# hwang595/ps_pytorch

Measured on AMD Instinct MI355X. Metric: images/sec (whole node), ResNet-18/CIFAR-10 synchronous PS training, higher is better.
Workload: dtype bf16; 1 GPU; model=ResNet18, global_batch=1024, input=3x32x32, per_worker_batch=1024, parallelism=single-gpu, engine=single-machine trainer (hipGraph-captured step), compress_grad=n/a (no comm at N=1), overlap=n/a (no comm at N=1)

## Files before the change

ps_pytorch_amd/ops/__init__.py:

```python
from __future__ import annotations

import ctypes
import os
from pathlib import Path
from typing import Optional

import torch

_LIB: Optional[ctypes.CDLL] = None
_LIB_ERR: Optional[str] = None

PS_F32 = 0
PS_BF16 = 1

_DTYPE_TAG = {torch.float32: PS_F32, torch.bfloat16: PS_BF16}

F32_SYMBOLS = (
    'ps_conv_fwd_f32', 'ps_conv_dgrad_f32', 'ps_conv_wgrad_f32',
    'ps_conv_bias_grad_f32',
    'ps_maxpool_fwd_f32', 'ps_maxpool_bwd_f32',
    'ps_gavgpool_fwd_f32', 'ps_gavgpool_bwd_f32',
    'ps_softmax_ce_fwd_f32', 'ps_softmax_ce_bwd_f32',
    'ps_ce_metrics_f32', 'ps_softmax_ce_fwd_metrics_f32',
)


def _so_path() -> Path:
    return Path(__file__).resolve().parent / "libps_hip.so"


def _try_load() -> None:
    global _LIB, _LIB_ERR
    if _LIB is not None or _LIB_ERR is not None:
        return
    p = _so_path()
    if not p.exists():
        _LIB_ERR = f"{p} not built (run ps_pytorch_amd.ops.build or __graft_entry__.build())"
        return
    try:
        lib = ctypes.CDLL(str(p))
        lib.ps_fused_sgd.argtypes = [
            ctypes.c_void_p, ctypes.c_void_p, ctypes.c_void_p, ctypes.c_void_p,
            ctypes.c_long, ctypes.c_float, ctypes.c_float, ctypes.c_float,
            ctypes.c_float, ctypes.c_int, ctypes.c_int, ctypes.c_int, ctypes.c_void_p]
        lib.ps_pack_bf16.argtypes = [ctypes.c_void_p, ctypes.c_void_p,
                                     ctypes.c_long, ctypes.c_void_p]
        lib.ps_unpack_bf16.argtypes = [ctypes.c_void_p, ctypes.c_void_p,
                                       ctypes.c_long, ctypes.c_void_p]
        lib.ps_pack_q8.argtypes = [ctypes.c_void_p, ctypes.c_void_p,
                                   ctypes.c_long, ctypes.c_int, ctypes.c_void_p]
        lib.ps_pack_q8_ef.argtypes = [ctypes.c_void_p, ctypes.c_void_p,
                                      ctypes.c_void_p, ctypes.c_long,
                                      ctypes.c_int, ctypes.c_void_p]
        lib.ps_pack_bf16_ef.argtypes = [ctypes.c_void_p, ctypes.c_void_p,
                                        ctypes.c_void_p, ctypes.c_long,
                                        ctypes.c_void_p]
        lib.ps_unpack_q8.argtypes = [ctypes.c_void_p, ctypes.c_void_p,
                                     ctypes.c_long, ctypes.c_int, ctypes.c_void_p]
        lib.ps_acc.argtypes = [ctypes.c_void_p, ctypes.c_void_p,
                               ctypes.c_long, ctypes.c_int, ctypes.c_void_p]
        lib.ps_pack_topk_ef.argtypes = [ctypes.c_void_p] * 3 + [
            ctypes.c_long, ctypes.c_int, ctypes.c_int, ctypes.c_void_p]
        lib.ps_pack_topk_ef.restype = ctypes.c_int
        lib.ps_unpack_topk.argtypes = [ctypes.c_void_p, ctypes.c_void_p,
                                       ctypes.c_long, ctypes.c_int,
                                       ctypes.c_int, ctypes.c_void_p]
        lib.ps_unpack_topk.restype = ctypes.c_int
        lib.ps_fanin_reduce.argtypes = [
            ctypes.c_void_p, ctypes.POINTER(ctypes.c_void_p), ctypes.c_int,
            ctypes.c_int, ctypes.c_int, ctypes.c_long, ctypes.c_void_p]
        lib.ps_fanin_reduce.restype = ctypes.c_int
        lib.ps_fanin_sgd.argtypes = [ctypes.c_void_p] * 3 + [
            ctypes.c_int, ctypes.POINTER(ctypes.c_void_p), ctypes.c_int,
            ctypes.c_int, ctypes.c_int, ctypes.c_long] + [
            ctypes.c_float] * 4 + [ctypes.c_int, ctypes.c_void_p]
        lib.ps_fanin_sgd.restype = ctypes.c_int
        lib.ps_conv_fwd.argtypes = [ctypes.c_void_p] * 5 + [ctypes.c_int] * 11 + [ctypes.c_void_p]
        lib.ps_conv_dgrad.argtypes = [ctypes.c_void_p] * 4 + [ctypes.c_int] * 11 + [ctypes.c_void_p]
        lib.ps_conv_wgrad.argtypes = [ctypes.c_void_p] * 4 + [ctypes.c_int] * 12 + [ctypes.c_void_p]
        lib.ps_conv_wgrad_row_variant.argtypes = [ctypes.c_void_p] * 3 + [
            ctypes.c_int] * 9 + [ctypes.c_void_p]
        lib.ps_conv_wgrad_row_variant.restype = ctypes.c_int
        lib.ps_conv_bias_grad.argtypes = [ctypes.c_void_p] * 3 + [
            ctypes.c_long, ctypes.c_int, ctypes.c_void_p]
        lib.ps_wt_transpose.argtypes = [ctypes.c_void_p, ctypes.c_void_p,
                                        ctypes.c_int, ctypes.c_int, ctypes.c_void_p]
        lib.ps_fused_adam.argtypes = [ctypes.c_void_p] * 6 + [
            ctypes.c_long] + [ctypes.c_float] * 7 + [
            ctypes.c_int, ctypes.c_int, ctypes.c_void_p]
        lib.ps_bn_fwd.argtypes = [ctypes.c_void_p] * 13 + [
            ctypes.c_int,
            ctypes.c_long, ctypes.c_long, ctypes.c_float, ctypes.c_float,
            ctypes.c_int, ctypes.c_int, ctypes.c_int, ctypes.c_void_p]
        lib.ps_bn_bwd.argtypes = [ctypes.c_void_p] * 12 + [
            ctypes.c_long, ctypes.c_long, ctypes.c_int, ctypes.c_int,
            ctypes.c_void_p]
        lib.ps_softmax_ce_fwd.argtypes = [ctypes.c_void_p] * 5 + [
            ctypes.c_long, ctypes.c_int, ctypes.c_void_p]
        lib.ps_softmax_ce_bwd.argtypes = [ctypes.c_void_p] * 5 + [
            ctypes.c_long, ctypes.c_int, ctypes.c_void_p]
        lib.ps_ce_metrics.argtypes = [ctypes.c_void_p] * 5 + [
            ctypes.c_long] + [ctypes.c_int] * 6 + [ctypes.c_void_p]
        lib.ps_softmax_ce_fwd_metrics.argtypes = [ctypes.c_void_p] * 7 + [
            ctypes.c_long] + [ctypes.c_int] * 6 + [ctypes.c_void_p]
        lib.ps_maxpool_fwd.argtypes = [ctypes.c_void_p] * 3 + [
            ctypes.c_int] * 10 + [ctypes.c_void_p]
        lib.ps_maxpool_bwd.argtypes = [ctypes.c_void_p] * 3 + [
            ctypes.c_int] * 10 + [ctypes.c_void_p]
        lib.ps_gavgpool_fwd.argtypes = [ctypes.c_void_p] * 2 + [
            ctypes.c_int] * 3 + [ctypes.c_void_p]
        lib.ps_gavgpool_bwd.argtypes = [ctypes.c_void_p] * 2 + [
            ctypes.c_int] * 3 + [ctypes.c_void_p]
        lib.ps_pad4.argtypes = [ctypes.c_void_p, ctypes.c_void_p,
                                ctypes.c_long, ctypes.c_int, ctypes.c_void_p]
        lib.ps_padc.argtypes = [ctypes.c_void_p, ctypes.c_void_p,
                                ctypes.c_long, ctypes.c_int, ctypes.c_int,
                                ctypes.c_void_p]
        lib.ps_act_drop_fwd.argtypes = [ctypes.c_void_p] * 3 + [
            ctypes.c_long, ctypes.c_int, ctypes.c_int, ctypes.c_uint32,
            ctypes.c_float, ctypes.c_uint64, ctypes.c_uint32,
            ctypes.c_void_p, ctypes.c_void_p]
        lib.ps_act_drop_bwd.argtypes = [ctypes.c_void_p] * 3 + [
            ctypes.c_long, ctypes.c_int, ctypes.c_float, ctypes.c_void_p]
        lib.ps_rng_advance.argtypes = [ctypes.c_void_p, ctypes.c_void_p]
        lib.ps_augment_batch.argtypes = [ctypes.c_void_p] * 5 + [
            ctypes.c_long] + [ctypes.c_int] * 7 + [
            ctypes.POINTER(ctypes.c_float), ctypes.POINTER(ctypes.c_float),
            ctypes.c_uint64, ctypes.c_uint32, ctypes.c_void_p,
            ctypes.c_void_p]
        lib.ps_conv_fwd_f32.argtypes = [ctypes.c_void_p] * 4 + [ctypes.c_int] * 11 + [ctypes.c_void_p]
        lib.ps_conv_dgrad_f32.argtypes = [ctypes.c_void_p] * 4 + [ctypes.c_int] * 11 + [ctypes.c_void_p]
        lib.ps_conv_wgrad_f32.argtypes = [ctypes.c_void_p] * 4 + [ctypes.c_int] * 12 + [ctypes.c_void_p]
        lib.ps_conv_bias_grad_f32.argtypes = [ctypes.c_void_p] * 3 + [
            ctypes.c_long, ctypes.c_int, ctypes.c_void_p]
        lib.ps_softmax_ce_fwd_f32.argtypes = lib.ps_softmax_ce_fwd.argtypes
        lib.ps_softmax_ce_bwd_f32.argtypes = lib.ps_softmax_ce_bwd.argtypes
        lib.ps_ce_metrics_f32.argtypes = lib.ps_ce_metrics.argtypes
        lib.ps_softmax_ce_fwd_metrics_f32.argtypes = \
            lib.ps_softmax_ce_fwd_metrics.argtypes
        lib.ps_maxpool_fwd_f32.argtypes = lib.ps_maxpool_fwd.argtypes
        lib.ps_maxpool_bwd_f32.argtypes = lib.ps_maxpool_bwd.argtypes
        lib.ps_gavgpool_fwd_f32.argtypes = lib.ps_gavgpool_fwd.argtypes
        lib.ps_gavgpool_bwd_f32.argtypes = lib.ps_gavgpool_bwd.argtypes
        _LIB = lib
    except OSError as e:
        _LIB_ERR = str(e)


def lib_or_none() -> Optional[ctypes.CDLL]:
    _try_load()
    return _LIB


def require_lib() -> ctypes.CDLL:
    _try_load()
    if _LIB is None:
        raise RuntimeError(
            f"ps_pytorch_amd HIP extension unavailable on a GPU host: {_LIB_ERR}")
    return _LIB


def dtype_tag(dt: torch.dtype) -> int:
    try:
        return _DTYPE_TAG[dt]
    except KeyError:
# ... 9 lines not shown
```

ps_pytorch_amd/ops/kernels/conv.hip:

```cpp
#include "common.h"
#include <stdlib.h>

typedef __bf16 bf16x8_t __attribute__((ext_vector_type(8)));
typedef unsigned short ushort8_t __attribute__((ext_vector_type(8)));
typedef float f32x4_t __attribute__((ext_vector_type(4)));

#define MFMA_BF16(a, b, c) __builtin_amdgcn_mfma_f32_16x16x32_bf16(a, b, c, 0, 0, 0)

union V16 {
    uint4 u4;
    unsigned short us[8];
    bf16x8_t bv;
};

__device__ __forceinline__ V16 zero16() {
    V16 v; v.u4 = make_uint4(0, 0, 0, 0); return v;
}

template <bool AL>
__device__ __forceinline__ V16 load16(const unsigned short* src, int cc, int Cn) {
    V16 v;
    if constexpr (AL) {
        v.u4 = *(const uint4*)src;
    } else if (cc + 8 <= Cn) {
// ... 408 lines not shown
            int col = n0 + segc;
            f32x4_t a0 = *(const f32x4_t*)&sf[rl * TN + segc];
            f32x4_t a1 = *(const f32x4_t*)&sf[rl * TN + segc + 4];
            float v[8];
#pragma unroll
            for (int k2 = 0; k2 < 4; ++k2) { v[k2] = a0[k2]; v[4 + k2] = a1[k2]; }
            if (vec_ok && col + 8 <= Nout) {
                V16 o;
                if constexpr (ACCF) {
                    V16 cv = *(const V16*)&carry[om * Nout + col];
#pragma unroll
                    for (int k2 = 0; k2 < 8; ++k2)
                        v[k2] += bf16_to_f32(cv.us[k2]);
                }
#pragma unroll
                for (int k2 = 0; k2 < 8; ++k2) o.us[k2] = f32_to_bf16(v[k2]);
                if constexpr (STATS)
#pragma unroll
                    for (int k2 = 0; k2 < 8; ++k2) {
                        float rv = bf16_to_f32(o.us[k2]);
                        ssum[k2] += rv;
                        ssq[k2] += rv * rv;
                    }
                *(uint4*)&dst[om * Nout + col] = o.u4;
            } else {
                for (int k2 = 0; k2 < 8 && col + k2 < Nout; ++k2) {
                    float vv = v[k2];
                    if constexpr (ACCF)
                        vv += bf16_to_f32(carry[om * Nout + col + k2]);
                    unsigned short ov = f32_to_bf16(vv);
                    if constexpr (STATS) {
                        float rv = bf16_to_f32(ov);
                        ssum[k2] += rv;
                        ssq[k2] += rv * rv;
                    }
                    dst[om * Nout + col + k2] = ov;
                }
            }
        }
        if constexpr (STATS) {
            __syncthreads();
            float* sp = sf;
#pragma unroll
            for (int k2 = 0; k2 < 8; ++k2) {
                sp[(rl0 * SEG + t % SEG) * 8 + k2] = ssum[k2];
                sp[(RPP * SEG + rl0 * SEG + t % SEG) * 8 + k2] = ssq[k2];
            }
            __syncthreads();
            if (rl0 == 0) {
                for (int rr2 = 1; rr2 < RPP; ++rr2)
#pragma unroll
                    for (int k2 = 0; k2 < 8; ++k2) {
                        ssum[k2] += sp[(rr2 * SEG + t % SEG) * 8 + k2];
                        ssq[k2] += sp[(RPP * SEG + rr2 * SEG + t % SEG) * 8 + k2];
                    }
                float* dst2 = stats + tile_m * 2 * (long)Nout + n0 + segc;
                for (int k2 = 0; k2 < 8 && n0 + segc + k2 < Nout; ++k2) {
                    dst2[k2] = ssum[k2];
                    dst2[Nout + k2] = ssq[k2];
                }
            }
        }
    } else {
#pragma unroll
    for (int nj = 0; nj < NJ; ++nj) {
        int col = n0 + wn * (NJ * 16) + nj * 16 + fr;
        float bv = (!DGRAD && bias && col < Nout) ? bf16_to_f32(bias[col]) : 0.f;
#pragma unroll
        for (int mi = 0; mi < 4; ++mi)
#pragma unroll
        for (int e = 0; e < 4; ++e) {
            long om = m0 + wm * 64 + mi * 16 + fq * 4 + e;
            if (om < M && col < Nout) {
                float v = acc[mi][nj][e] + bv;
                if constexpr (ACCF)
                    v += bf16_to_f32(carry[om * Nout + col]);
                dst[om * Nout + col] = f32_to_bf16(v);
            }
        }
    }
    }
}

template <int TM, int TN, bool AL = true, int SWZM = 2, bool ACCF = false>
__global__ __launch_bounds__(256) void conv_dgrad2_kernel(
    const unsigned short* __restrict__ dout,
    const unsigned short* __restrict__ wgt,
    unsigned short* __restrict__ dx,
    const unsigned short* __restrict__ carry,
    int Nb, int H, int W, int C, int K, int P, int Q,
    int R, int S, int pad, int4 ends, int4 codes)
{
    int bx = blockIdx.x;
    int cls;
    if      (bx < ends.x) cls = 0;
    else if (bx < ends.y) { cls = 1; bx -= ends.x; }
    else if (bx < ends.z) { cls = 2; bx -= ends.y; }
    else                  { cls = 3; bx -= ends.z; }
    const int code = (cls == 0) ? codes.x : (cls == 1) ? codes.y
                     : (cls == 2) ? codes.z : codes.w;
    const int hp = code >> 1, wp = code & 1;
    const int Hc = (H - hp + 1) >> 1, Wc = (W - wp + 1) >> 1;
    __shared__ __attribute__((aligned(16))) FwdLds<TM, TN> lds;
    constexpr int SWZ = SWZM;
    constexpr int AR = TM / 32;
    constexpr int BR = TN / 32;
    const long M = (long)Nb * Hc * Wc;
    const int tiles_n = (C + TN - 1) / TN;
    const long m0 = (bx / tiles_n) * (long)TM;
    const int n0 = (bx % tiles_n) * TN;
    const int t = threadIdx.x;
    const int trow = t >> 3;
    const int cc8 = (t & 7) * 8;

    const int r0 = (hp + pad) & 1, s0 = (wp + pad) & 1;
    const int nr = (R > r0) ? ((R - r0 + 1) >> 1) : 0;
    const int ns = (S > s0) ? ((S - s0 + 1) >> 1) : 0;

    const unsigned short* pA[AR];
    unsigned int vm[AR];
#pragma unroll
    for (int rr = 0; rr < AR; ++rr) {
        long m = m0 + trow + 32 * rr;
        pA[rr] = dout; vm[rr] = 0;
        if (m < M) {
            int n = (int)(m / ((long)Hc * Wc)); int rem = (int)(m % ((long)Hc * Wc));
            int h = hp + 2 * (rem / Wc), w = wp + 2 * (rem % Wc);
            int p1 = (h + pad - r0) >> 1, q1 = (w + pad - s0) >> 1;
            pA[rr] = dout + (long)n * P * Q * K + ((long)p1 * Q + q1) * K + cc8;
            unsigned int msk = 0;
            for (int ri = 0; ri < nr; ++ri)
                for (int si = 0; si < ns; ++si)
                    if (p1 - ri >= 0 && p1 - ri < P
                        && q1 - si >= 0 && q1 - si < Q)
                        msk |= 1u << (ri * ns + si);
            vm[rr] = msk;
        }
    }

    constexpr int WGM = TM / 64;
    constexpr int WGN = 4 / WGM;
    constexpr int NJ = TN / WGN / 16;
    const int lane = t & 63, wid = t >> 6;
    const int wm = (WGN == 1) ? wid : (wid >> 1);
    const int wn = (WGN == 1) ? 0 : (wid & 1);
    const int fr = lane & 15, fq = lane >> 4;
    f32x4_t acc[4][NJ];
#pragma unroll
    for (int i = 0; i < 4; ++i)
#pragma unroll
        for (int j = 0; j < NJ; ++j) acc[i][j] = {0.f, 0.f, 0.f, 0.f};

    const int KC = (K + 63) >> 6;
    const int KCm1 = (KC - 1) * 64;
    const int nsteps = nr * ns * KC;
    int lsi = 0, lkc = 0;
    V16 areg[AR], breg[BR];

    const unsigned short* pB[BR];
    bool colv[BR];
#pragma unroll
    for (int rr = 0; rr < BR; ++rr) {
        int col = n0 + trow + 32 * rr;
        colv[rr] = col < C;
        pB[rr] = wgt + (((long)(r0 * S + s0) * C) + (colv[rr] ? col : 0))
                 * (long)K + cc8;
// ... 498 lines not shown
#pragma unroll
            for (int mi = 0; mi < MI; ++mi)
#pragma unroll
                for (int nj = 0; nj < 2; ++nj)
                    acc[s][mi][nj] = MFMA_BF16(a[mi].v, bf[nj].v,
                                               acc[s][mi][nj]);
        }
    };

    load_step();
    write_lds(0);
    if (nsteps > 1) load_step();
    __syncthreads();
    int it = 0;
    for (; it + 3 < nsteps; it += 2) {
        write_lds(1);
        load_step();
        mfma_step(0);
        __syncthreads();
        write_lds(0);
        load_step();
        mfma_step(1);
        __syncthreads();
    }
    const int rem = nsteps - it;
    if (rem >= 2) {
        write_lds(1);
        if (rem >= 3) load_step();
    }
    if (rem >= 1) mfma_step(0);
    if (rem >= 2) {
        __syncthreads();
        if (rem >= 3) write_lds(0);
        mfma_step(1);
    }
    if (rem >= 3) {
        __syncthreads();
        mfma_step(0);
    }

    const int RSC = 9 * C;
    float* dstp = partial + (long)sid * K * RSC;
#pragma unroll
    for (int s = 0; s < 3; ++s)
#pragma unroll
    for (int mi = 0; mi < MI; ++mi)
#pragma unroll
    for (int nj = 0; nj < 2; ++nj)
#pragma unroll
    for (int e = 0; e < 4; ++e) {
        int k = k0 + wm * (MI * 16) + mi * 16 + fq * 4 + e;
        int c = c0 + wn * 32 + nj * 16 + fr;
        if (k < K && c < C)
            dstp[(long)k * RSC + (r * 3 + s) * C + c] = acc[s][mi][nj][e];
    }
}


__device__ __forceinline__ int wrho(int e) {
    return (((e >> 1) & 1) + ((e >> 3) & 1) * 2) << 1;
}

#define WG_RING_NST 4

struct WgRingStage {
    unsigned short A[32][64];
    unsigned short B[64][64];
};

__device__ __forceinline__ void wg_ring_dma3(
    const void* g0, const void* g1, const void* g2,
    unsigned l0, unsigned l1, unsigned l2)
{
    unsigned keep;
    asm volatile(
        "s_mov_b32 %0, m0\n\t"
        "s_mov_b32 m0, %4\n\ts_nop 0\n\tglobal_load_lds_dwordx4 %1, off\n\t"
        "s_mov_b32 m0, %5\n\ts_nop 0\n\tglobal_load_lds_dwordx4 %2, off\n\t"
        "s_mov_b32 m0, %6\n\ts_nop 0\n\tglobal_load_lds_dwordx4 %3, off\n\t"
        "s_mov_b32 m0, %0"
        : "=&s"(keep)
        : "v"(g0), "v"(g1), "v"(g2), "s"(l0), "s"(l1), "s"(l2)
        : "memory");
}

template <int N>
__device__ __forceinline__ void wg_ring_sync() {
    asm volatile("s_waitcnt vmcnt(%0)\n\ts_waitcnt lgkmcnt(0)\n\ts_barrier"
                 :: "i"(N) : "memory");
}

template <int NST>
__global__ __launch_bounds__(256) void conv_wgrad_row_ring_kernel(
    const unsigned short* __restrict__ dout,
    const unsigned short* __restrict__ in,
    float* __restrict__ partial,
    const unsigned short* __restrict__ zpage,
    int Nb, int H, int W, int C, int K, int P, int Q,
    int split, int ipr, int l2q, int l2p, int per_xcd)
{
    static_assert(NST == 3 || NST == 4, "ring depth");
    constexpr int TK = 64;
    constexpr int PAD = 1;
    constexpr int DPS = 3;
    const int ROWS = 32 >> l2q;
    const int HW2 = W + 2;
    __shared__ __attribute__((aligned(16))) WgRingStage sg0, sg1, sg2, sg3;
    auto stg = [&](int st) -> WgRingStage* {
        return st == 0 ? &sg0 : st == 1 ? &sg1 : st == 2 ? &sg2 : &sg3;
    };
    constexpr int MI = TK / 32;
    const int tiles_k = (K + TK - 1) / TK;
    const int tiles_c = (C + 63) >> 6;
    long l = (long)(blockIdx.x & 7) * per_xcd + (blockIdx.x >> 3);
    const long nlog = (long)tiles_k * tiles_c * 3 * split;
    if (l >= nlog) return;
    int b = (int)l;
    const int k0 = (b % tiles_k) * TK; b /= tiles_k;
    const int c0 = (b % tiles_c) * 64; b /= tiles_c;
    const int r = b % 3; b /= 3;
    const int sid = b;
    const long rows_total = (long)Nb * P;
    const long row0 = (long)sid * ipr;
    const long row1 = (row0 + ipr < rows_total) ? row0 + ipr : rows_total;

    const int t = threadIdx.x;
    const int lane = t & 63, wid = t >> 6;
    const int wm = wid >> 1, wn = wid & 1;
    const int fr = lane & 15, fq = lane >> 4;
    f32x4_t acc[3][MI][2];
#pragma unroll
    for (int si = 0; si < 3; ++si)
#pragma unroll
        for (int i = 0; i < MI; ++i)
#pragma unroll
            for (int j = 0; j < 2; ++j) acc[si][i][j] = {0.f, 0.f, 0.f, 0.f};

    const int nsteps = (int)((row1 - row0 + (1 << (5 - l2q)) - 1)
                             >> (5 - l2q));

    const int apix = wid * 8 + (lane >> 3);
    const int aoct = ((lane & 7) ^ wrho(apix));
    const unsigned short* pdout = dout + (row0 << l2q) * K + k0;
    const int a_off = apix * K + aoct * 8;
    const int a_row = apix >> l2q;
    const long inrow0 = row0 + r - PAD;
    const unsigned short* pin0 = in + inrow0 * W * C + c0;
    int b_rib[2], b_off[2];
    bool b_wok[2];
#pragma unroll
    for (int j = 0; j < 2; ++j) {
        int hp = wid * 16 + j * 8 + (lane >> 3);
        int oct = ((lane & 7) ^ wrho(hp));
        b_rib[j] = hp / HW2;
        int wpx = hp - b_rib[j] * HW2 - 1;
        b_wok[j] = wpx >= 0 && wpx < W && hp < ROWS * HW2;
        b_off[j] = (b_rib[j] * W + (wpx < 0 ? 0 : wpx)) * C + oct * 8;
    }
    long prow = row0;

    const unsigned wu = (unsigned)__builtin_amdgcn_readfirstlane(wid);
    const unsigned ldA = wu * (8 * 128);
    const unsigned ldB = (unsigned)sizeof(sg0.A) + wu * (16 * 128);

    auto dma_stage = [&](int st) {
        const unsigned sb = (unsigned)(unsigned long)
            (__attribute__((address_space(3))) void*)stg(st);
        const unsigned short* gs[DPS];
        const long rl = rows_total - prow;
        const int rleft = rl < 64 ? (int)rl : 64;
        const int pl = (int)prow;
        gs[0] = a_row < rleft ? pdout + a_off : zpage;
#pragma unroll
        for (int j = 0; j < 2; ++j) {
            int h = ((pl + b_rib[j]) & (P - 1)) + r - PAD;
            bool ok = b_wok[j] & ((unsigned)h < (unsigned)H)
                      & (b_rib[j] < rleft);
            gs[1 + j] = ok ? pin0 + b_off[j] : zpage;
        }
        wg_ring_dma3(gs[0], gs[1], gs[2],
                     sb + ldA, sb + ldB, sb + ldB + 8 * 128);
        pdout += (long)32 * K;
        pin0 += (long)ROWS * W * C;
        prow += ROWS;
    };

    const char* lb0 = (const char*)&sg0;
    unsigned roA[MI][2];
    unsigned roB[3][2][2];
#pragma unroll
    for (int i = 0; i < 2; ++i) {
        int e = fq * 8 + i * 4 + (fr >> 2);
        int qd = fr & 3;
#pragma unroll
        for (int mi = 0; mi < MI; ++mi) {
            int o = (wm * MI + mi) * 2 + (qd >> 1);
            roA[mi][i] = (unsigned)((char*)&sg0.A[e]
                             [(o ^ wrho(e)) * 8 + (qd & 1) * 4] - lb0);
        }
        int rib = e >> l2q, q = e & (Q - 1);
#pragma unroll
        for (int si = 0; si < 3; ++si) {
            int hp = rib * HW2 + q + si;
#pragma unroll
            for (int nj = 0; nj < 2; ++nj) {
                int o = (wn * 2 + nj) * 2 + (qd >> 1);
                roB[si][nj][i] = (unsigned)((char*)&sg0.B[hp]
                                 [(o ^ wrho(hp)) * 8 + (qd & 1) * 4] - lb0);
            }
        }
    }

    union U64x8 { bf16x4_t h[2]; bf16x8_t v; };
    auto mfma_step = [&](int st) {
        const char* sbp = (const char*)stg(st);
        U64x8 a[MI];
#pragma unroll
        for (int mi = 0; mi < MI; ++mi) {
            a[mi].h[0] = ds_tr16p((const unsigned short*)
                (sbp + roA[mi][0]));
            a[mi].h[1] = ds_tr16p((const unsigned short*)
                (sbp + roA[mi][1]));
        }
#pragma unroll
        for (int si = 0; si < 3; ++si) {
            U64x8 bf[2];
#pragma unroll
            for (int nj = 0; nj < 2; ++nj) {
                bf[nj].h[0] = ds_tr16p((const unsigned short*)
                    (sbp + roB[si][nj][0]));
                bf[nj].h[1] = ds_tr16p((const unsigned short*)
                    (sbp + roB[si][nj][1]));
            }
#pragma unroll
            for (int mi = 0; mi < MI; ++mi)
#pragma unroll
                for (int nj = 0; nj < 2; ++nj)
                    acc[si][mi][nj] = MFMA_BF16(a[mi].v, bf[nj].v,
                                                acc[si][mi][nj]);
        }
    };

    auto ring_sync = [&](int ahead) {
        if (NST > 3 && ahead >= 2) wg_ring_sync<2 * DPS>();
        else if (ahead >= 1)       wg_ring_sync<DPS>();
        else                       wg_ring_sync<0>();
    };

#pragma unroll
    for (int j = 0; j < NST - 1; ++j)
        if (j < nsteps) dma_stage(j);
    int it = 0;
    for (; it + 2 * NST - 2 < nsteps; it += NST) {
#pragma unroll
        for (int j = 0; j < NST; ++j) {
            ring_sync(NST - 2);
            dma_stage((j + NST - 1) % NST);
            mfma_step(j);
        }
    }
    const int rem = nsteps - it;
#pragma unroll
    for (int j = 0; j < 2 * NST - 2; ++j) {
        if (j < rem) {
            const int left = rem - 1 - j;
            ring_sync(left < NST - 2 ? left : NST - 2);
            if (j + NST - 1 < rem) dma_stage((j + NST - 1) % NST);
            mfma_step(j % NST);
        }
    }

    const int RSC = 9 * C;
    float* dstp = partial + (long)sid * K * RSC;
#pragma unroll
    for (int si = 0; si < 3; ++si)
#pragma unroll
    for (int mi = 0; mi < MI; ++mi)
#pragma unroll
    for (int nj = 0; nj < 2; ++nj)
#pragma unroll
    for (int e = 0; e < 4; ++e) {
        int k = k0 + wm * (MI * 16) + mi * 16 + fq * 4 + e;
        int c = c0 + wn * 32 + nj * 16 + fr;
        if (k < K && c < C)
            dstp[(long)k * RSC + (r * 3 + si) * C + c] = acc[si][mi][nj][e];
    }
}

template <int STRIDE, bool POW2, bool AL = true, int CPM = 0>
__global__ __launch_bounds__(256) void conv_wgrad_small_kernel(
    const unsigned short* __restrict__ dout,
    const unsigned short* __restrict__ in,
    float* __restrict__ partial,
    int Nb, int H, int W, int C, int K, int P, int Q,
    int R, int S, int pad, int split, int chunk,
    int l2pq, int l2q,
    unsigned long long mpq, unsigned long long mq)
{
    __shared__ __attribute__((aligned(16))) WgradLds<64> lds;
    const long M = (long)Nb * P * Q;
    const int RSC = R * S * C;
    const int tiles_k = (K + 63) >> 6;
    const int nc = (RSC + 63) >> 6;
    int b = blockIdx.x;
    const int k0 = (b % tiles_k) * 64; b /= tiles_k;
    const int e0 = (b % nc) * 64; b /= nc;
    const int sid = b;
    const long mbeg = (long)sid * chunk;
    const long mend = (mbeg + chunk < M) ? mbeg + chunk : M;

    const int t = threadIdx.x;
    const int trow = t >> 3;
    const int cc8 = (t & 7) * 8;
    const int lane = t & 63, wid = t >> 6;
    const int wm = wid >> 1, wn = wid & 1;
    const int fr = lane & 15, fq = lane >> 4;
    f32x4_t acc[2][2];
#pragma unroll
    for (int i = 0; i < 2; ++i)
#pragma unroll
        for (int j = 0; j < 2; ++j) acc[i][j] = {0.f, 0.f, 0.f, 0.f};

    int tre[8], tse[8], toff[8];
#pragma unroll
    for (int u = 0; u < 8; ++u) {
        int e = e0 + cc8 + u;
        if constexpr (CPM == 8) {
            int tp = e / C;
            tre[u] = tp / S;
// ... 351 lines not shown
    int vec_ok = (((uintptr_t)dst | (uintptr_t)src) & 15) == 0;
    int blocks;
    ew_grid(vec_ok ? ((n + 7) >> 3) / PS_SEED_U + 1 : n, 256, &blocks);
    hipLaunchKernelGGL(seed_dx_kernel<PS_SEED_U>, dim3(blocks), dim3(256), 0,
                       (hipStream_t)strm, (unsigned short*)dst,
                       (const unsigned short*)src, n, vec_ok);
}


static inline int swz_mode() {
    static int m = -1;
    if (m < 0) { const char* e = getenv("PS_SWZ"); m = e ? atoi(e) : 2; }
    return m;
}

static inline int glds_mode() {
    static int m = -1;
    if (m < 0) { const char* e = getenv("PS_GLDS"); m = e ? atoi(e) : 1; }
    return m;
}

static const unsigned short* zpage_ptr() {
    static const unsigned short* z = [] {
        void* p = nullptr;
        (void)hipMalloc(&p, 128);
        (void)hipMemset(p, 0, 128);
        return (const unsigned short*)p;
    }();
    return z;
}

#define LAUNCH_GEMM(TM, TN, ST, DG, SM) LAUNCH_GEMM_NB(TM, TN, ST, DG, SM, 2)
#define LAUNCH_GEMM_NB(TM, TN, ST, DG, SM, NBV)                               \
    do {                                                                      \
        if (swz_mode() == 1) LAUNCH_GEMM_SW(TM, TN, ST, DG, SM, NBV, 1, false); \
        else                 LAUNCH_GEMM_SW(TM, TN, ST, DG, SM, NBV, 2, false); \
    } while (0)
#define LAUNCH_GEMM_ACC(TM, TN, ST, DG, SM, ACV)                              \
    do {                                                                      \
        if (swz_mode() == 1) LAUNCH_GEMM_SW(TM, TN, ST, DG, SM, 2, 1, ACV);   \
        else                 LAUNCH_GEMM_SW(TM, TN, ST, DG, SM, 2, 2, ACV);   \
    } while (0)
#define LAUNCH_GEMM_CV(TM, TN, ST, SM, NBV) LAUNCH_GEMM_CP(TM, TN, ST, SM, NBV, 4)
#define LAUNCH_GEMM_CP(TM, TN, ST, SM, NBV, CPV)                              \
    do {                                                                      \
        long M_ = (long)Nb * P * Q;                                           \
        long grid = ((M_ + TM - 1) / TM) * ((K + TN - 1) / TN);               \
        hipLaunchKernelGGL((conv_gemm_kernel<TM, TN, ST, false, SM, ALV, NBV, \
                                             2, false, CPV>),               \
            dim3((unsigned)grid), dim3(256), 0, (hipStream_t)strm,            \
            (const unsigned short*)src, (const unsigned short*)wgt,           \
            (const unsigned short*)bias, (unsigned short*)dst,                \
            (const unsigned short*)carry, nullptr, nullptr,                   \
            Nb, H, W, C, K, P, Q, R, S, pad);                                 \
    } while (0)
#define LAUNCH_GEMM_GLS(TM, TN, ST, DG, SM, NBV, SWV, ACV, GLV, STV)          \
    do {                                                                      \
        long M_ = DG ? (long)Nb * H * W : (long)Nb * P * Q;                   \
        int Nout_ = DG ? C : K;                                               \
        long grid = ((M_ + TM - 1) / TM) * ((Nout_ + TN - 1) / TN);           \
        hipLaunchKernelGGL((conv_gemm_kernel<TM, TN, ST, DG, SM, ALV, NBV,    \
                                             SWV, ACV, 0, GLV, STV>),         \
            dim3((unsigned)grid), dim3(256), 0, (hipStream_t)strm,            \
            (const unsigned short*)src, (const unsigned short*)wgt,           \
            (const unsigned short*)bias, (unsigned short*)dst,                \
            (const unsigned short*)carry, zpage_ptr(), (float*)stats,         \
            Nb, H, W, C, K, P, Q, R, S, pad);                                 \
    } while (0)
#define LAUNCH_GEMM_GL(TM, TN, ST, DG, SM, NBV, SWV, ACV, GLV)                \
    do {                                                                      \
        if (!(DG) && stats) LAUNCH_GEMM_GLS(TM, TN, ST, DG, SM, NBV, SWV, ACV, GLV, true); \
        else                LAUNCH_GEMM_GLS(TM, TN, ST, DG, SM, NBV, SWV, ACV, GLV, false); \
    } while (0)
#define LAUNCH_GEMM_SW(TM, TN, ST, DG, SM, NBV, SWV, ACV)                     \
    do {                                                                      \
        if constexpr (ALV && !(SM)) {                                         \
            if (glds_mode()) LAUNCH_GEMM_GL(TM, TN, ST, DG, SM, NBV, SWV, ACV, true); \
            else             LAUNCH_GEMM_GL(TM, TN, ST, DG, SM, NBV, SWV, ACV, false); \
        } else {                                                              \
            LAUNCH_GEMM_GL(TM, TN, ST, DG, SM, NBV, SWV, ACV, false);         \
        }                                                                     \
    } while (0)

extern "C" void ps_conv_fwd(
    const void* src, const void* wgt, const void* bias, void* dst,
    void* stats,
    int Nb, int H, int W, int C, int K, int P, int Q,
    int R, int S, int stride, int pad, void* strm)
{
    const void* carry = nullptr;
    bool al = (C & 63) == 0;
#define FWD_BODY()                                                            \
    do {                                                                      \
        if (R * S > 1 && C == 4 && R * S * 4 <= 64) {        \
            if (K <= 32) {            \
                if (stride == 1) LAUNCH_GEMM_CV(128, 32, 1, true, 1);         \
                else             LAUNCH_GEMM_CV(128, 32, 2, true, 1);         \
            } else if (stride == 1) LAUNCH_GEMM_CV(128, 64, 1, true, 1);      \
            else             LAUNCH_GEMM_CV(128, 64, 2, true, 1);             \
        } else if (R * S > 1 && C == 4 && R * S * 4 <= 256) {                 \
            if (K <= 32) {                                                    \
                if (stride == 1) LAUNCH_GEMM_CV(128, 32, 1, true, 2);         \
                else             LAUNCH_GEMM_CV(128, 32, 2, true, 2);         \
            } else if (stride == 1) LAUNCH_GEMM_CV(128, 64, 1, true, 2);      \
            else             LAUNCH_GEMM_CV(128, 64, 2, true, 2);             \
        } else if (R * S > 1 && (C & 7) == 0 && (C & 63)                      \
                   && R * S * C <= 768) {              \
            if (K <= 32) {                                                    \
                if (stride == 1) LAUNCH_GEMM_CP(128, 32, 1, true, 2, 8);      \
                else             LAUNCH_GEMM_CP(128, 32, 2, true, 2, 8);      \
            } else if (stride == 1) LAUNCH_GEMM_CP(128, 64, 1, true, 2, 8);   \
            else             LAUNCH_GEMM_CP(128, 64, 2, true, 2, 8);          \
        } else if (R * S > 1 && R * S * C <= 64) {    \
            if (stride == 1) LAUNCH_GEMM_NB(128, 64, 1, false, true, 1);      \
            else             LAUNCH_GEMM_NB(128, 64, 2, false, true, 1);      \
        } else if (R * S > 1 && R * S * C <= 192) {                           \
            if (stride == 1) LAUNCH_GEMM(128, 64, 1, false, true);            \
            else             LAUNCH_GEMM(128, 64, 2, false, true);            \
        } else if (R * S == 1 && C <= 64) {              \
            if (stride == 1) LAUNCH_GEMM_NB(128, 64, 1, false, false, 1);     \
            else             LAUNCH_GEMM_NB(128, 64, 2, false, false, 1);     \
        } else if (K >= 128) {                                                \
            if (stride == 1) LAUNCH_GEMM(128, 128, 1, false, false);          \
            else             LAUNCH_GEMM(128, 128, 2, false, false);          \
        } else if (K <= 32) {         \
            if (stride == 1) LAUNCH_GEMM(128, 32, 1, false, false);           \
            else             LAUNCH_GEMM(128, 32, 2, false, false);           \
        } else {                                                              \
            if (stride == 1) LAUNCH_GEMM(128, 64, 1, false, false);           \
            else             LAUNCH_GEMM(128, 64, 2, false, false);           \
        }                                                                     \
    } while (0)
    if (al) { constexpr bool ALV = true; FWD_BODY(); }
    else    { constexpr bool ALV = false; FWD_BODY(); }
#undef FWD_BODY
}

extern "C" void ps_conv_dgrad(
    const void* src, const void* wgt, void* dst, const void* carry,
    int Nb, int H, int W, int C, int K, int P, int Q,
    int R, int S, int stride, int pad, void* strm)
{
    const void* bias = nullptr;
    const void* stats = nullptr;
    bool al = (K & 63) == 0;
    if (stride == 1) {
#define DG_BODY(ACV)                                                          \
        do {                                                                  \
            if (C >= 128)     LAUNCH_GEMM_ACC(128, 128, 1, true, false, ACV); \
            else if (C <= 32) LAUNCH_GEMM_ACC(128, 32, 1, true, false, ACV);  \
            else              LAUNCH_GEMM_ACC(128, 64, 1, true, false, ACV);  \
        } while (0)
        if (al) { constexpr bool ALV = true;
                  if (carry) DG_BODY(true); else DG_BODY(false); }
        else    { constexpr bool ALV = false;
                  if (carry) DG_BODY(true); else DG_BODY(false); }
#undef DG_BODY
    } else {
        const unsigned short* dout = (const unsigned short*)src;
        bool any_empty = false;
        for (int hp = 0; hp < 2 && hp < H; ++hp)
        for (int wp = 0; wp < 2 && wp < W; ++wp) {
            int r0 = (hp + pad) & 1, s0 = (wp + pad) & 1;
            if (R <= r0 || S <= s0) any_empty = true;
        }
        if (any_empty)
            launch_seed_dx(dst, carry, (long)Nb * H * W * C, strm);
        int TM_ = 128, TN_ = (C >= 128) ? 128 : 64;
        int tiles_n_ = (C + TN_ - 1) / TN_;
        int ends_[4] = {0, 0, 0, 0}, codes_[4] = {0, 0, 0, 0};
        int slot = 0, total = 0;
        for (int hp = 0; hp < 2 && hp < H; ++hp)
        for (int wp = 0; wp < 2 && wp < W; ++wp) {
            int r0 = (hp + pad) & 1, s0 = (wp + pad) & 1;
            if (R <= r0 || S <= s0) continue;
            int Hc = (H - hp + 1) >> 1, Wc = (W - wp + 1) >> 1;
            long M_ = (long)Nb * Hc * Wc;
            total += (int)(((M_ + TM_ - 1) / TM_) * tiles_n_);
            ends_[slot] = total;
            codes_[slot] = (hp << 1) | wp;
            ++slot;
        }
        for (int i = slot; i < 4; ++i) { ends_[i] = total; codes_[i] = 0; }
        if (total == 0) return;
        int4 ends = make_int4(ends_[0], ends_[1], ends_[2], ends_[3]);
        int4 codes = make_int4(codes_[0], codes_[1], codes_[2], codes_[3]);
#define DG2_SW(TM, TN, ALV, SWV, ACV)                                         \
        hipLaunchKernelGGL((conv_dgrad2_kernel<TM, TN, ALV, SWV, ACV>),       \
            dim3((unsigned)total), dim3(256), 0, (hipStream_t)strm, dout,     \
            (const unsigned short*)wgt, (unsigned short*)dst,                 \
            (const unsigned short*)carry,                                     \
            Nb, H, W, C, K, P, Q, R, S, pad, ends, codes)
#define DG2_AC(TM, TN, ALV, SWV) do {                                         \
        if (carry) DG2_SW(TM, TN, ALV, SWV, true);                            \
        else       DG2_SW(TM, TN, ALV, SWV, false); } while (0)
#define DG2(TM, TN, ALV) do {                                                 \
        if (swz_mode() == 1) DG2_AC(TM, TN, ALV, 1);                          \
        else                 DG2_AC(TM, TN, ALV, 2); } while (0)
        if (al) { if (C >= 128) DG2(128, 128, true);
                  else          DG2(128, 64, true); }
        else    { if (C >= 128) DG2(128, 128, false);
                  else          DG2(128, 64, false); }
#undef DG2
    }
}

static inline int ilog2_exact(long v) {
    int l = 0; while ((1L << l) < v) ++l;
    return ((1L << l) == v) ? l : -1;
}

static bool wgrad_row_eligible(int H, int W, int C, int K, int P, int Q,
                               int variant)
{
    if (P != H || Q != W || ilog2_exact(Q) < 0 || ilog2_exact(P) < 0
        || Q < 4 || Q > 32)
        return false;
    if (variant == 1) return (C & 63) == 0 && (K & 63) == 0;
    return variant == 0;
}

static void launch_wgrad_row(
    const void* dout, const void* in, void* partial_f32,
    int Nb, int H, int W, int C, int K, int P, int Q, int split,
    int variant, void* strm)
{
    const int TKr = 64;
    int l2q_ = ilog2_exact(Q);
    int tkr = (K + TKr - 1) / TKr, tcr = (C + 63) / 64;
    long rows_total = (long)Nb * P;
    int ROWS = 32 >> l2q_;
    long ipr_l = (rows_total + split - 1) / split;
    ipr_l = ((ipr_l + ROWS - 1) / ROWS) * ROWS;
    long nlog = (long)tkr * tcr * 3 * split;
    int pxc = (int)((nlog + 7) / 8);
    long grid_r = (long)pxc * 8;
    bool alr = ((C & 63) == 0) && (K % TKr == 0);
#define WGR(TKV, ALV)                                                         \
    hipLaunchKernelGGL((conv_wgrad_row_kernel<TKV, ALV>),                     \
        dim3((unsigned)grid_r), dim3(256), 0, (hipStream_t)strm,              \
        (const unsigned short*)dout, (const unsigned short*)in,               \
        (float*)partial_f32, Nb, H, W, C, K, P, Q,                            \
        split, (int)ipr_l, l2q_, 0, pxc)
    if (variant == 1)
        hipLaunchKernelGGL((conv_wgrad_row_ring_kernel<WG_RING_NST>),
            dim3((unsigned)grid_r), dim3(256), 0, (hipStream_t)strm,
            (const unsigned short*)dout, (const unsigned short*)in,
            (float*)partial_f32, zpage_ptr(), Nb, H, W, C, K, P, Q,
            split, (int)ipr_l, l2q_, 0, pxc);
    else if (alr) WGR(64, true);
    else          WGR(64, false);
#undef WGR
}

extern "C" int ps_conv_wgrad_row_variant(
    const void* dout, const void* in, void* partial_f32,
    int Nb, int H, int W, int C, int K, int P, int Q, int split,
    int variant, void* strm)
{
    if (split < 1 || Nb < 1
        || !wgrad_row_eligible(H, W, C, K, P, Q, variant))
        return 1;
    launch_wgrad_row(dout, in, partial_f32, Nb, H, W, C, K, P, Q, split,
                     variant, strm);
    return 0;
}

extern "C" void ps_conv_wgrad(
    const void* dout, const void* in, void* partial_f32, void* dw,
    int Nb, int H, int W, int C, int K, int P, int Q,
    int R, int S, int stride, int pad, int split, void* strm)
{
    long M = (long)Nb * P * Q;
    long chunk64 = (M + (long)split * 64 - 1) / ((long)split * 64);
    int chunk = (int)(chunk64 * 64);
    if (R * S > 1 && ((C == 4 && R * S * 4 <= 256)
                      || ((C & 7) == 0 && (C & 63) && R * S * C <= 768)
                      || R * S * C <= 192)) {
        int tiles_k = (K + 63) / 64;
        int nc_s = (R * S * C + 63) / 64;
        long grid_s = (long)tiles_k * nc_s * split;
        int l2pq_ = ilog2_exact((long)P * Q), l2q_ = ilog2_exact(Q);
        bool pw = l2pq_ >= 0 && l2q_ >= 0;
        unsigned long long mpq_ = fdiv_magic((long)P * Q);
        unsigned long long mq_ = fdiv_magic(Q);
#define WGS(ST, PW, CV)                                                       \
        hipLaunchKernelGGL((conv_wgrad_small_kernel<ST, PW, false, CV>),      \
// ... 115 lines not shown
```

Baseline: 130,300 images/sec.

## Add halo-tiled 3x3 conv kernel for 64-channel fwd and dgrad

Adds a dedicated 3x3 stride-1 conv kernel for C=K=64 layers at 16 or 32 width. It loads each 128-pixel output tile plus its one-pixel halo into LDS once through direct global-to-LDS DMA, then reuses that tile across all nine taps. Weight taps stream through a three-slot ring buffer overlapped with the MFMA work. This replaces the generic implicit-GEMM path, which re-gathers input for every tap. The cost is extra code, LDS pressure that may limit occupancy, and a new path selected by default through an env var.

```diff
diff --git a/ps_pytorch_amd/ops/__init__.py b/ps_pytorch_amd/ops/__init__.py
--- a/ps_pytorch_amd/ops/__init__.py
+++ b/ps_pytorch_amd/ops/__init__.py
@@ -81,6 +81,9 @@
         lib.ps_conv_wgrad_row_variant.argtypes = [ctypes.c_void_p] * 3 + [
             ctypes.c_int] * 9 + [ctypes.c_void_p]
         lib.ps_conv_wgrad_row_variant.restype = ctypes.c_int
+        lib.ps_conv_halo_variant.argtypes = [ctypes.c_int] + [
+            ctypes.c_void_p] * 5 + [ctypes.c_int] * 8 + [ctypes.c_void_p]
+        lib.ps_conv_halo_variant.restype = ctypes.c_int
         lib.ps_conv_bias_grad.argtypes = [ctypes.c_void_p] * 3 + [
             ctypes.c_long, ctypes.c_int, ctypes.c_void_p]
         lib.ps_wt_transpose.argtypes = [ctypes.c_void_p, ctypes.c_void_p,
diff --git a/ps_pytorch_amd/ops/kernels/conv.hip b/ps_pytorch_amd/ops/kernels/conv.hip
--- a/ps_pytorch_amd/ops/kernels/conv.hip
+++ b/ps_pytorch_amd/ops/kernels/conv.hip
@@ -514,6 +514,201 @@
     }
 }
 
+template <int W>
+struct HaloLds {
+    static constexpr int RT = 128 / W;
+    static constexpr int HW2 = W + 2;
+    static constexpr int NPIX = (RT + 2) * HW2;
+    static constexpr int PW = (NPIX + 31) / 32;
+    unsigned short A[PW * 32][64];
+    unsigned short B[3][64][64];
+};
+
+__device__ __forceinline__ void halo_dma1(const void* g0, unsigned l0)
+{
+    unsigned keep;
+    asm volatile(
+        "s_mov_b32 %0, m0\n\t"
+        "s_mov_b32 m0, %2\n\ts_nop 0\n\tglobal_load_lds_dwordx4 %1, off\n\t"
+        "s_mov_b32 m0, %0"
+        : "=&s"(keep) : "v"(g0), "s"(l0) : "memory");
+}
+
+__device__ __forceinline__ void halo_dma2(
+    const void* g0, const void* g1, unsigned l0, unsigned l1)
+{
+    unsigned keep;
+    asm volatile(
+        "s_mov_b32 %0, m0\n\t"
+        "s_mov_b32 m0, %3\n\ts_nop 0\n\tglobal_load_lds_dwordx4 %1, off\n\t"
+        "s_mov_b32 m0, %4\n\ts_nop 0\n\tglobal_load_lds_dwordx4 %2, off\n\t"
+        "s_mov_b32 m0, %0"
+        : "=&s"(keep) : "v"(g0), "v"(g1), "s"(l0), "s"(l1) : "memory");
+}
+
+template <int N>
+__device__ __forceinline__ void lds_ring_sync() {
+    asm volatile("s_waitcnt vmcnt(%0)\n\ts_waitcnt lgkmcnt(0)\n\ts_barrier"
+                 :: "i"(N) : "memory");
+}
+
+template <int W, bool DGRAD, bool ACCF>
+__global__ __launch_bounds__(256) void conv3x3_halo_kernel(
+    const unsigned short* __restrict__ src,
+    const unsigned short* __restrict__ wgt,
+    const unsigned short* __restrict__ bias,
+    unsigned short* __restrict__ dst,
+    const unsigned short* __restrict__ carry,
+    const unsigned short* __restrict__ zpage,
+    int H)
+{
+    using L = HaloLds<W>;
+    constexpr int RT = L::RT, HW2 = L::HW2, NPIX = L::NPIX, PW = L::PW;
+    constexpr int J0 = 5;
+    static_assert(RT * HW2 <= 32 * J0 && 32 * PW - 2 * HW2 <= 32 * J0
+                  && J0 <= PW, "early-start piece count");
+    static_assert(sizeof(L) >= 128 * 64 * 4, "f32 staging fits LDS");
+    __shared__ __attribute__((aligned(128))) L lds;
+
+    const int t = threadIdx.x;
+    const int lane = t & 63, wid = t >> 6;
+    const int wm = wid >> 1, wn = wid & 1;
+    const int fr = lane & 15, fq = lane >> 4;
+    const int tpi = H / RT;
+    const int n = blockIdx.x / tpi;
+    const int h0 = (blockIdx.x - n * tpi) * RT;
+    const long m0 = (long)blockIdx.x * 128;
+    const unsigned short* img = src + (long)n * H * W * 64;
+
+    const int wu = __builtin_amdgcn_readfirstlane(wid);
+    const unsigned ldsA = (unsigned)(unsigned long)
+        (__attribute__((address_space(3))) void*)&lds.A[0][0];
+    const unsigned ldsB = (unsigned)(unsigned long)
+        (__attribute__((address_space(3))) void*)&lds.B[0][0][0];
+
+    const unsigned short* pB[2];
+#pragma unroll
+    for (int rr = 0; rr < 2; ++rr) {
+        int row = wid * 16 + rr * 8 + (lane >> 3);
+        pB[rr] = wgt + row * (DGRAD ? 64 : 9 * 64)
+                 + gswz<2>(row, lane & 7) * 8;
+    }
+    constexpr int BTAP = DGRAD ? 64 * 64 : 64;
+    auto dma_b = [&](int tap) {
+        const unsigned l = ldsB + (tap % 3) * 8192 + wu * 2048;
+        halo_dma2(pB[0] + tap * BTAP, pB[1] + tap * BTAP, l, l + 1024);
+    };
+    auto dma_a = [&](int j) {
+        const int i = j * 4 + wu;
+        const int gi = DGRAD ? 4 * PW - 1 - i : i;
+        const int lp = gi * 8 + (lane >> 3);
+        const int hr = lp / HW2, hc = lp - hr * HW2;
+        const int h = h0 - 1 + hr, wc = hc - 1;
+        const bool ok = (lp < NPIX) & ((unsigned)h < (unsigned)H)
+                        & ((unsigned)wc < (unsigned)W);
+        const int off = (h * W + wc) * 64
+                        + (((lane & 7) ^ (((lp >> 1) & 3) << 1)) * 8);
+        const unsigned short* gs = ok ? img + off : zpage;
+        halo_dma1(gs, ldsA + gi * 1024);
+    };
+
+    f32x4_t acc[4][2];
+#pragma unroll
+    for (int i = 0; i < 4; ++i)
+#pragma unroll
+        for (int j = 0; j < 2; ++j) acc[i][j] = {0.f, 0.f, 0.f, 0.f};
+
+    int lp0[4];
+#pragma unroll
+    for (int mi = 0; mi < 4; ++mi) {
+        int o = wm * 64 + mi * 16 + fr;
+        lp0[mi] = (o / W) * HW2 + (o % W);
+    }
+    int brow[2];
+#pragma unroll
+    for (int nj = 0; nj < 2; ++nj) brow[nj] = wn * 32 + nj * 16 + fr;
+
+    auto mfma_tap = [&](int tap) {
+        const int r = tap / 3, s = tap % 3;
+        const int toff = DGRAD ? (2 - r) * HW2 + (2 - s) : r * HW2 + s;
+#pragma unroll
+        for (int kk = 0; kk < 2; ++kk) {
+            bf16x8_t a[4], b[2];
+#pragma unroll
+            for (int mi = 0; mi < 4; ++mi) {
+                int lp = lp0[mi] + toff;
+                a[mi] = *(const bf16x8_t*)
+                    &lds.A[lp][((kk * 4 + fq) ^ (((lp >> 1) & 3) << 1)) * 8];
+            }
+#pragma unroll
+            for (int nj = 0; nj < 2; ++nj)
+                b[nj] = *(const bf16x8_t*)
+                    &lds.B[tap % 3][brow[nj]]
+                          [gswz<2>(brow[nj], kk * 4 + fq) * 8];
+#pragma unroll
+            for (int mi = 0; mi < 4; ++mi)
+#pragma unroll
+                for (int nj = 0; nj < 2; ++nj)
+                    acc[mi][nj] = MFMA_BF16(a[mi], b[nj], acc[mi][nj]);
+        }
+    };
+
+    dma_b(0);
+#pragma unroll
+    for (int j = 0; j < J0; ++j) dma_a(j);
+    dma_b(1);
+#pragma unroll
+    for (int j = J0; j < PW; ++j) dma_a(j);
+    dma_b(2);
+
+#pragma unroll
+    for (int tap = 0; tap < 9; ++tap) {
+        if (tap == 0)      lds_ring_sync<PW - J0 + 4>();
+        else if (tap == 1) lds_ring_sync<PW - J0 + 2>();
+        else if (tap < 8)  lds_ring_sync<2>();
+        else               lds_ring_sync<0>();
+        if (tap >= 1 && tap + 2 < 9) dma_b(tap + 2);
+        mfma_tap(tap);
+    }
+    lds_ring_sync<0>();
+
+    float* sf = reinterpret_cast<float*>(&lds);
+#pragma unroll
+    for (int nj = 0; nj < 2; ++nj) {
+        int cl = wn * 32 + nj * 16 + fr;
+        float bv = (!DGRAD && bias) ? bf16_to_f32(bias[cl]) : 0.f;
+#pragma unroll
+        for (int mi = 0; mi < 4; ++mi)
+#pragma unroll
+        for (int e = 0; e < 4; ++e)
+            sf[(wm * 64 + mi * 16 + fq * 4 + e) * 64 + cl]
+                = acc[mi][nj][e] + bv;
+    }
+    __syncthreads();
+    const int segc = (t & 7) * 8;
+    const int rl0 = t >> 3;
+#pragma unroll
+    for (int ps = 0; ps < 4; ++ps) {
+        int rl = ps * 32 + rl0;
+        long om = m0 + rl;
+        f32x4_t a0 = *(const f32x4_t*)&sf[rl * 64 + segc];
+        f32x4_t a1 = *(const f32x4_t*)&sf[rl * 64 + segc + 4];
+        float v[8];
+#pragma unroll
+        for (int k2 = 0; k2 < 4; ++k2) { v[k2] = a0[k2]; v[4 + k2] = a1[k2]; }
+        V16 o;
+        if constexpr (ACCF) {
+            V16 cv = *(const V16*)&carry[om * 64 + segc];
+#pragma unroll
+            for (int k2 = 0; k2 < 8; ++k2)
+                v[k2] += bf16_to_f32(cv.us[k2]);
+        }
+#pragma unroll
+        for (int k2 = 0; k2 < 8; ++k2) o.us[k2] = f32_to_bf16(v[k2]);
+        *(uint4*)&dst[om * 64 + segc] = o.u4;
+    }
+}
+
 template <int TM, int TN, bool AL = true, int SWZM = 2, bool ACCF = false>
 __global__ __launch_bounds__(256) void conv_dgrad2_kernel(
     const unsigned short* __restrict__ dout,
@@ -1178,12 +1373,6 @@
         : "=&s"(keep)
         : "v"(g0), "v"(g1), "v"(g2), "s"(l0), "s"(l1), "s"(l2)
         : "memory");
-}
-
-template <int N>
-__device__ __forceinline__ void wg_ring_sync() {
-    asm volatile("s_waitcnt vmcnt(%0)\n\ts_waitcnt lgkmcnt(0)\n\ts_barrier"
-                 :: "i"(N) : "memory");
 }
 
 template <int NST>
@@ -1338,9 +1527,9 @@
     };
 
     auto ring_sync = [&](int ahead) {
-        if (NST > 3 && ahead >= 2) wg_ring_sync<2 * DPS>();
-        else if (ahead >= 1)       wg_ring_sync<DPS>();
-        else                       wg_ring_sync<0>();
+        if (NST > 3 && ahead >= 2) lds_ring_sync<2 * DPS>();
+        else if (ahead >= 1)       lds_ring_sync<DPS>();
+        else                       lds_ring_sync<0>();
     };
 
 #pragma unroll
@@ -1858,7 +2047,7 @@
         }                                                                     \
     } while (0)
 
-extern "C" void ps_conv_fwd(
+static void conv_fwd_generic(
     const void* src, const void* wgt, const void* bias, void* dst,
     void* stats,
     int Nb, int H, int W, int C, int K, int P, int Q,
@@ -1912,7 +2101,7 @@
 #undef FWD_BODY
 }
 
-extern "C" void ps_conv_dgrad(
+static void conv_dgrad_generic(
     const void* src, const void* wgt, void* dst, const void* carry,
     int Nb, int H, int W, int C, int K, int P, int Q,
     int R, int S, int stride, int pad, void* strm)
@@ -1979,6 +2168,92 @@
                   else          DG2(128, 64, false); }
 #undef DG2
     }
+}
+
+static inline int halo_mode() {
+    static int m = -1;
+    if (m < 0) { const char* e = getenv("PS_CONV_HALO"); m = e ? atoi(e) : 1; }
+    return m;
+}
+
+static bool conv_halo_eligible(int H, int W, int C, int K, int P, int Q,
+                               int R, int S, int stride, int pad,
+                               const void* stats)
+{
+    return R == 3 && S == 3 && stride == 1 && pad == 1 && P == H && Q == W
+        && C == 64 && K == 64 && (W == 16 || W == 32) && H > 0
+        && H % (128 / W) == 0 && stats == nullptr;
+}
+
+static void launch_conv_halo(
+    bool dgrad, const void* src, const void* wgt, const void* bias,
+    void* dst, const void* carry, int Nb, int H, int W, void* strm)
+{
+    const long grid = (long)Nb * H * W / 128;
+#define HALO(WV, DG, ACV)                                                     \
+    hipLaunchKernelGGL((conv3x3_halo_kernel<WV, DG, ACV>),                    \
+        dim3((unsigned)grid), dim3(256), 0, (hipStream_t)strm,                \
+        (const unsigned short*)src, (const unsigned short*)wgt,               \
+        (const unsigned short*)bias, (unsigned short*)dst,                    \
+        (const unsigned short*)carry, zpage_ptr(), H)
+#define HALO_W(DG, ACV) do { if (W == 32) HALO(32, DG, ACV);                  \
+                             else         HALO(16, DG, ACV); } while (0)
+    if (!dgrad)     HALO_W(false, false);
+    else if (carry) HALO_W(true, true);
+    else            HALO_W(true, false);
+#undef HALO_W
+#undef HALO
+}
+
+static inline bool halo_on() {
+    return halo_mode() && glds_mode() && swz_mode() == 2;
+}
+
+extern "C" void ps_conv_fwd(
+    const void* src, const void* wgt, const void* bias, void* dst,
+    void* stats,
+    int Nb, int H, int W, int C, int K, int P, int Q,
+    int R, int S, int stride, int pad, void* strm)
+{
+    if (halo_on()
+        && conv_halo_eligible(H, W, C, K, P, Q, R, S, stride, pad, stats))
+        launch_conv_halo(false, src, wgt, bias, dst, nullptr, Nb, H, W, strm);
+    else
+        conv_fwd_generic(src, wgt, bias, dst, stats, Nb, H, W, C, K, P, Q,
+                         R, S, stride, pad, strm);
+}
+
+extern "C" void ps_conv_dgrad(
+    const void* src, const void* wgt, void* dst, const void* carry,
+    int Nb, int H, int W, int C, int K, int P, int Q,
+    int R, int S, int stride, int pad, void* strm)
+{
+    if (halo_on()
+        && conv_halo_eligible(H, W, C, K, P, Q, R, S, stride, pad, nullptr))
+        launch_conv_halo(true, src, wgt, nullptr, dst, carry, Nb, H, W, strm);
+    else
+        conv_dgrad_generic(src, wgt, dst, carry, Nb, H, W, C, K, P, Q,
+                           R, S, stride, pad, strm);
+}
+
+extern "C" int ps_conv_halo_variant(
+    int dgrad, const void* src, const void* wgt, const void* bias,
+    void* dst, const void* carry,
+    int Nb, int H, int W, int C, int K, int P, int Q, int variant, void* strm)
+{
+    if (Nb < 1 || (variant != 0 && variant != 1)
+        || !conv_halo_eligible(H, W, C, K, P, Q, 3, 3, 1, 1, nullptr))
+        return 1;
+    if (variant == 1)
+        launch_conv_halo(dgrad != 0, src, wgt, dgrad ? nullptr : bias, dst,
+                         dgrad ? carry : nullptr, Nb, H, W, strm);
+    else if (dgrad)
+        conv_dgrad_generic(src, wgt, dst, carry, Nb, H, W, C, K, P, Q,
+                           3, 3, 1, 1, strm);
+    else
+        conv_fwd_generic(src, wgt, bias, dst, nullptr, Nb, H, W, C, K, P, Q,
+                         3, 3, 1, 1, strm);
+    return 0;
 }
 
 static inline int ilog2_exact(long v) {
```

Measured after the change: 140,000 images/sec, median of 6. 1.07x the previous value.
